# SandeepaInduwaraSamaranayake/SwinVox

Measured on AMD Instinct MI355X. Metric: views/sec fwd+bwd SwinVox-T 224^2, 32^3 voxel, n_views=8, higher is better.
Workload: dtype bf16; 1 GPU; SwinVox-T full pipeline (ResNet50[:layer3] || Swin multi-stage, cross-view attention, decoder, merger, refiner), fwd+2xBCE+bwd, train mode, B=64 samples x V=8 views of 224x224 per GPU; global_batch=64, n_views=8, images_per_gpu=512, parallelism=single GPU, launch=eager (one host launch per kernel, three streams)

## Files before the change

include/swinvox_hip.h:

```cpp
#ifndef SWINVOX_HIP_H
#define SWINVOX_HIP_H
#include <stddef.h>
#include <stdint.h>

#ifdef __cplusplus
extern "C" {
#endif

#define SV_OK 0
#define SV_ERR_INVALID (-1)
#define SV_ERR_LAUNCH (-2)

enum { SV_ACT_NONE = 0, SV_ACT_RELU = 1, SV_ACT_GELU = 2, SV_ACT_LRELU = 3 };
#define SV_BN_SLOTS 16
enum { SV_MATH_F32 = 0, SV_MATH_BF16 = 1, SV_MATH_FP8 = 2, SV_MATH_FP8_FULL = 3 };
enum { SV_F32 = 0, SV_BF16 = 1 };

const char* sv_last_error(void);
int sv_version(void);

typedef struct sv_geom {
  int N;
  int Di, Hi, Wi;
  int Do, Ho, Wo;
  int Ci, Co;
  int kd, kh, kw;
  int sd, sh, sw;
  int pd, ph, pw;
  int ldi;
} sv_geom;

typedef struct sv_epilogue {
  const float* bias;
  const void* residual;
  int ldr;
  const float* row_scale;
  int rows_per_scale;
  void* pre_act;
  double* stats;
  int act;
  float slope;
  const void* act_grad_src;
  int act_grad_kind;
  int ldc;
  int col_off;
} sv_epilogue;

int sv_conv_gather(const void* in, const void* w_packed, void* out, const sv_geom* g, const sv_epilogue* e,
                   int math, int act_dtype, void* stream);
int sv_set_conv_halo(int mode);
int sv_conv_halo_mode(void);
int sv_set_conv_halo_wgrad(int mode);
long long sv_conv_halo_launches(void);
enum { SV_PATH_GATHER = 0,
       SV_PATH_DENSE = 1,
       SV_PATH_WIDE = 2,
       SV_PATH_WIDE_GENERAL = 3,
       SV_PATH_HALO0 = 4, SV_PATH_HALO1 = 5, SV_PATH_HALO2 = 6,
       SV_PATH_HALO_BLOCKED_8X32 = 7, SV_PATH_HALO_BLOCKED_16X16 = 8,
       SV_PATH_WGRAD_TILED = 9,
       SV_PATH_WGRAD_WIDE = 10, SV_PATH_WGRAD_WIDE_SWAP = 11,
       SV_PATH_WGRAD_HALO = 12 };
enum { SV_OPERANDS_F32 = 0, SV_OPERANDS_BF16_F32 = 1, SV_OPERANDS_BF16 = 2 };
typedef struct sv_launch_plan {
  int path;
  int tile_rows, tile_cols;
  int operands;
  int vec;
  int grid_x, grid_y, block;
} sv_launch_plan;
int sv_conv_gather_plan(const void* in, const void* w, void* out, const sv_geom* g, const sv_epilogue* e, int math, int act_dtype, int transposed,
                        sv_launch_plan* plan);
int sv_conv_gather_is_wide(const void* in, const void* w, void* out, const sv_geom* g, const sv_epilogue* e, int math, int act_dtype);
int sv_tconv_gather(const void* in, const void* w_packed, void* out, const sv_geom* g, const sv_epilogue* e,
                    int math, int act_dtype, void* stream);
int sv_conv_wgrad_plan(const void* anchor, int lda, const void* gathered, const sv_geom* g, int cg_valid, int math, int act_dtype,
                       sv_launch_plan* plan);
int sv_conv_wgrad_is_wide(const void* anchor, int lda, const void* gathered, const sv_geom* g, int cg_valid, int math, int act_dtype);
size_t sv_conv_wgrad_workspace_floats(const sv_geom* g);
int sv_conv_wgrad(const void* anchor, int lda, const void* gathered, float* dw, const sv_geom* g, int cg_valid,
                  float* workspace, float* dbias , int math, int act_dtype,
                  void* stream);
int sv_quant_rows_e4m3(const void* src, int src_dtype, int rows, int K, int ld, void* dst_q, int Kp, float* scales, void* stream);
int sv_linear_fp8(const void* xq, const float* sx, const void* wq, const float* sw, void* out, int M, int K, int N, const sv_epilogue* e,
                  int act_dtype, void* stream);
int sv_linear_fp8_supported(int K, int N, const sv_epilogue* e, int math, int act_dtype);
long long sv_linear_fp8_launches(void);
int sv_quant_cols_e4m3(const void* src, int src_dtype, int M, int C, int ld, void* dst_q, int Mp, float* scales, float* colsum, void* stream);
int sv_linear_fp8_dgrad(const void* dq, const float* sd, const void* wtq, const float* swt, void* dx, int M, int N, int K, const sv_epilogue* e,
                        int act_dtype, void* stream);
int sv_linear_fp8_dgrad_supported(int N, int K, const sv_epilogue* e, int math, int act_dtype);
int sv_linear_fp8_wgrad(const void* dyt, const float* sdc, const void* xt, const float* sxc, float* dw, int M, int N, int K, int ldw, int splits,
                        void* stream);
long long sv_linear_fp8_bwd_launches(int which);
int sv_quant_rows_mx_e4m3(const void* src, int src_dtype, int rows, int K, int ld, void* dst_q, int Kp, void* scales_u8, void* stream);
int sv_linear_mxfp8(const void* xq, const void* xs, const void* wq, const void* ws, void* out, int M, int K, int N, const sv_epilogue* e,
                    void* q_out, void* qs_out, int act_dtype, void* stream);
long long sv_linear_mxfp8_launches(void);
long long sv_quant_rows_mx_launches(void);
int sv_quant_cols_mx_e4m3(const void* src, int src_dtype, int M, int C, int ld, void* dst_q, int Mp, void* scales_u8, float* colsum, void* stream);
int sv_linear_mxfp8_dgrad(const void* dq, const void* ds, const void* wtq, const void* wts, void* dx, int M, int N, int K, const sv_epilogue* e,
                          int act_dtype, void* stream);
size_t sv_linear_mxfp8_wgrad_workspace_floats(int M, int N, int K, int splits);
int sv_linear_mxfp8_wgrad(const void* dyt, const void* dys, const void* xt, const void* xs, float* dw, int M, int N, int K, int ldw, int splits,
                          float* workspace, void* stream);
long long sv_linear_mxfp8_bwd_launches(int which);
long long sv_quant_cols_mx_launches(void);
int sv_mx_rows_to_cols(const void* xq, int Kp, const void* xs, int M, int K, void* dst_q, int Mp, void* scales_u8, void* stream);
long long sv_mx_rows_to_cols_launches(void);
int sv_quant_rows_cols_mx_e4m3(const void* src, int src_dtype, int M, int N, int ld, void* row_q, int Np, void* row_s, void* col_q, int Mp,
                               void* col_s, float* colsum, void* stream);
long long sv_quant_rows_cols_mx_launches(void);
int sv_stencil3_fwd(const void* x, int ldx, int cin_load, int groups, const void* w_bf16, int ntiles16,
                    const float* bias, void* out, int ldc, int col_off, int cout, const void* residual, int ldr,
                    double* stats, int I, int D, int H, int W, long long x_plane_stride, long long out_plane_stride, int act_dtype,
                    void* stream);
size_t sv_stencil3_wgrad_workspace_floats(int cout, int cin);
int sv_stencil3_wgrad(const void* x, int ldx, int cin_load, int groups, const void* dy, int lddy, int cout_load,
                      float* dw, float* dbias, float* workspace, int cout, int cin, int c_stride, int c_valid, int I, int D, int H, int W,
                      long long x_plane_stride, int act_dtype, void* stream);
int sv_tconv4s2_fwd(const void* x, const void* w_packed, const float* bias, void* out, double* stats, int I, int D, int H, int W,
                    int cin, int cout, void* stream);
int sv_pack_weight(const float* src, void* dst, int A, int B, int T, int swap, int pad_to, int out_dtype, void* stream);
typedef struct sv_pack_desc {
  const float* src; void* dst;
  int A, B, T, swap, rows_out, inner_out, block0, reserved;
} sv_pack_desc;
int sv_pack_weights_block_elems(void);
int sv_pack_weights(const sv_pack_desc* descs_dev, int n, int total_blocks, int out_dtype, void* stream);
int sv_colsum(const void* x, int rows, int cols, int ld, float* out, int accumulate, int act_dtype, void* stream);
int sv_cast(const void* src, int src_dtype, void* dst, int dst_dtype, long long n, void* stream);

int sv_layernorm_fwd(const void* x, const float* gamma, const float* beta, void* y, float* mean, float* rstd,
                     long long rows, int C, float eps, int merge_H, int merge_W, int act_dtype, void* stream);
int sv_layernorm_quant_fwd(const void* x, const float* gamma, const float* beta, void* y, float* mean, float* rstd,
                           void* q, int Kp, float* scales, long long rows, int C, float eps, int merge_H, int merge_W,
                           int act_dtype, void* stream);
long long sv_layernorm_quant_launches(void);
int sv_layernorm_quant_mx_fwd(const void* x, const float* gamma, const float* beta, void* y, float* mean, float* rstd,
                              void* q, int Kp, void* scales_u8, long long rows, int C, float eps,
                              int merge_H, int merge_W, int act_dtype, void* stream);
long long sv_layernorm_quant_mx_launches(void);
size_t sv_layernorm_bwd_workspace_floats(int C);
int sv_layernorm_bwd(const void* dy, const void* x, const float* gamma, const float* mean, const float* rstd,
                     void* dx, float* dgamma, float* dbeta, float* workspace, long long rows, int C, int merge_H, int merge_W,
                     int accumulate_dx, int act_dtype, void* stream);
size_t sv_ln_image_workspace_floats(int I, int L);
int sv_ln_image_fwd(const void* x, const float* w, const float* b, void* y, float* meanrstd, float* workspace,
                    int I, int L, float eps, float drop_p, uint32_t seed, const uint32_t* seed_epoch, int act_dtype, void* stream);
int sv_ln_image_bwd(const void* dy, const void* x, const float* w, const float* meanrstd, void* dx, float* dw,
                    float* db, double* sums_ws , int I, int L, float drop_p, uint32_t seed,
                    const uint32_t* seed_epoch, int act_dtype, void* stream);
int sv_bn_stats(const void* x, long long M, int C, int ld, double* sums, int act_dtype, void* stream);
int sv_bn_finalize(const double* sums, long long count, const float* gamma, const float* beta, float* running_mean,
                   float* running_var, float momentum, float eps, int training, float* scale, float* shift,
                   float* save_mean, float* save_rstd, int C, void* stream);
int sv_scale_shift_act(const void* x, int ldx, const float* scale, const float* shift, const void* residual, int ldr,
                       void* y, int ldy, long long M, int C, int act, float slope, int act_dtype, void* stream);
int sv_bn_act_maxpool_fwd(const void* x, const float* scale, const float* shift, void* pooled, void* idx, int N, int H, int W, int C,
                          int act, float slope, int act_dtype, void* stream);
int sv_bn_maxpool_bwd(const void* dpooled, const void* idx, const void* x, const float* gamma, const float* save_mean, const float* save_rstd,
                      const float* fwd_scale, const float* fwd_shift, int N, int H, int W, int C, int act, float slope, int training,
                      void* dx, float* dgamma, float* dbeta, double* sums_ws, int act_dtype, void* stream);
int sv_bn_act_maxpool3d_fwd(const void* x, const float* scale, const float* shift, void* pooled, void* idx, int N, int D, int H, int W, int C,
                            int act, float slope, int act_dtype, void* stream);
// ... 153 lines not shown
```

swinvox_amd/hip.py:

```python
from __future__ import annotations

import ctypes as C
import os
import threading

import torch

_HERE = os.path.dirname(os.path.abspath(__file__))
LIB_PATH = os.environ.get("SV_HIP_LIB") or os.path.join(_HERE, "libswinvox_hip.so")

ACT_NONE, ACT_RELU, ACT_GELU, ACT_LRELU = 0, 1, 2, 3
MATH_F32, MATH_BF16, MATH_FP8, MATH_FP8_FULL = 0, 1, 2, 3
F32, BF16 = 0, 1


class Geom(C.Structure):
    _fields_ = [(n, C.c_int) for n in ("N", "Di", "Hi", "Wi", "Do", "Ho", "Wo", "Ci", "Co", "kd", "kh", "kw",
                                        "sd", "sh", "sw", "pd", "ph", "pw", "ldi")]


class Epilogue(C.Structure):
    _fields_ = [("bias", C.c_void_p), ("residual", C.c_void_p), ("ldr", C.c_int), ("row_scale", C.c_void_p),
                ("rows_per_scale", C.c_int), ("pre_act", C.c_void_p), ("stats", C.c_void_p), ("act", C.c_int),
                ("slope", C.c_float), ("act_grad_src", C.c_void_p), ("act_grad_kind", C.c_int), ("ldc", C.c_int),
                ("col_off", C.c_int)]


class LaunchPlan(C.Structure):
    _fields_ = [(n, C.c_int) for n in ("path", "tile_rows", "tile_cols", "operands", "vec", "grid_x", "grid_y", "block")]


(PATH_GATHER, PATH_DENSE, PATH_WIDE, PATH_WIDE_GENERAL, PATH_HALO0, PATH_HALO1, PATH_HALO2, PATH_HALO_BLOCKED_8X32, PATH_HALO_BLOCKED_16X16,
 PATH_WGRAD_TILED, PATH_WGRAD_WIDE, PATH_WGRAD_WIDE_SWAP, PATH_WGRAD_HALO) = range(13)
OPERANDS_F32, OPERANDS_BF16_F32, OPERANDS_BF16 = 0, 1, 2


class PackDesc(C.Structure):
    _fields_ = [("src", C.c_void_p), ("dst", C.c_void_p), ("A", C.c_int), ("B", C.c_int), ("T", C.c_int), ("swap", C.c_int),
                ("rows_out", C.c_int), ("inner_out", C.c_int), ("block0", C.c_int), ("reserved", C.c_int)]


class AugSample(C.Structure):
    _fields_ = [("bg", C.c_float * 3), ("jitter_value", C.c_float * 3), ("jitter_order", C.c_int * 3), ("noise", C.c_float * 3),
                ("perm", C.c_int * 3), ("mean", C.c_float * 3), ("std", C.c_float * 3)]


_P, _I, _L, _F, _U, _D = C.c_void_p, C.c_int, C.c_longlong, C.c_float, C.c_uint32, C.c_double
_ACT_TYPED = {
    "sv_conv_gather", "sv_tconv_gather", "sv_conv_wgrad", "sv_stencil3_fwd", "sv_stencil3_wgrad", "sv_colsum",
    "sv_layernorm_fwd", "sv_layernorm_quant_fwd", "sv_layernorm_quant_mx_fwd", "sv_layernorm_bwd", "sv_ln_image_fwd", "sv_ln_image_bwd", "sv_bn_stats", "sv_scale_shift_act", "sv_bn_bwd", "sv_scale_shift_act_signs", "sv_bn_bwd_signs", "sv_scale_shift_act2_signs", "sv_bn_bwd2_signs",
    "sv_window_attention_fwd", "sv_window_attention_fwd_mxq", "sv_window_attention_bwd", "sv_cross_view_attention_fwd", "sv_cross_view_attention_bwd",
    "sv_transpose", "sv_add_n", "sv_axpby", "sv_relu_bwd", "sv_maxpool2d_fwd", "sv_maxpool2d_bwd", "sv_avgpool2_fwd", "sv_avgpool2_bwd",
    "sv_decoder_seed_fwd", "sv_decoder_seed_bwd", "sv_maxpool3d_fwd", "sv_maxpool3d_bwd", "sv_dropout", "sv_rowscale",
    "sv_dwconv2x2_fwd", "sv_dwconv2x2_bwd", "sv_upsample3to7_add_fwd", "sv_upsample3to7_bwd",
    "sv_cva_downsample_fwd", "sv_cva_downsample_bwd", "sv_cva_upsample_add_fwd", "sv_cva_upsample_bwd", "sv_decoder_head_fwd", "sv_decoder_head_bwd",
    "sv_merge_views_fwd", "sv_merge_views_bwd", "sv_stem_space_to_depth", "sv_encoder_prep", "sv_encoder_prep_bwd", "sv_bn_act_maxpool_fwd", "sv_bn_maxpool_bwd", "sv_bn_act_maxpool3d_fwd", "sv_bn_maxpool3d_bwd", "sv_head_pack_x", "sv_head_unpack_dx", "sv_swin_attn_block_fwd", "sv_swin_attn_block_fwd_mx", "sv_swin_attn_block_bwd",
    "sv_linear_fp8", "sv_linear_fp8_dgrad", "sv_linear_mxfp8", "sv_linear_mxfp8_dgrad",
}
_PROTOS = {
    "sv_version": (_I, None),
    "sv_conv_gather": (_I, [_P, _P, _P, C.POINTER(Geom), C.POINTER(Epilogue), _I]),
    "sv_tconv_gather": (_I, [_P, _P, _P, C.POINTER(Geom), C.POINTER(Epilogue), _I]),
    "sv_conv_gather_plan": (_I, None, [_P, _P, _P, C.POINTER(Geom), C.POINTER(Epilogue), _I, _I, _I, C.POINTER(LaunchPlan)]),
    "sv_conv_gather_is_wide": (_I, None, [_P, _P, _P, C.POINTER(Geom), C.POINTER(Epilogue), _I, _I]),
    "sv_conv_wgrad_plan": (_I, None, [_P, _I, _P, C.POINTER(Geom), _I, _I, _I, C.POINTER(LaunchPlan)]),
    "sv_conv_wgrad_is_wide": (_I, None, [_P, _I, _P, C.POINTER(Geom), _I, _I, _I]),
    "sv_conv_wgrad_workspace_floats": (C.c_size_t, None, [C.POINTER(Geom)]),
    "sv_conv_wgrad": (_I, [_P, _I, _P, _P, C.POINTER(Geom), _I, _P, _P, _I]),
    "sv_quant_rows_e4m3": (_I, [_P, _I, _I, _I, _I, _P, _I, _P]),
    "sv_linear_fp8": (_I, [_P, _P, _P, _P, _P, _I, _I, _I, C.POINTER(Epilogue)]),
    "sv_linear_fp8_supported": (_I, None, [_I, _I, C.POINTER(Epilogue), _I, _I]),
    "sv_linear_fp8_launches": (_L, None),
    "sv_quant_cols_e4m3": (_I, [_P, _I, _I, _I, _I, _P, _I, _P, _P]),
    "sv_linear_fp8_dgrad": (_I, [_P, _P, _P, _P, _P, _I, _I, _I, C.POINTER(Epilogue)]),
    "sv_linear_fp8_dgrad_supported": (_I, None, [_I, _I, C.POINTER(Epilogue), _I, _I]),
    "sv_linear_fp8_wgrad": (_I, [_P, _P, _P, _P, _P, _I, _I, _I, _I, _I]),
    "sv_linear_fp8_bwd_launches": (_L, None, [_I]),
    "sv_quant_rows_mx_e4m3": (_I, [_P, _I, _I, _I, _I, _P, _I, _P]),
    "sv_linear_mxfp8": (_I, [_P, _P, _P, _P, _P, _I, _I, _I, C.POINTER(Epilogue), _P, _P]),
    "sv_linear_mxfp8_launches": (_L, None),
    "sv_quant_rows_mx_launches": (_L, None),
    "sv_quant_cols_mx_e4m3": (_I, [_P, _I, _I, _I, _I, _P, _I, _P, _P]),
    "sv_linear_mxfp8_dgrad": (_I, [_P, _P, _P, _P, _P, _I, _I, _I, C.POINTER(Epilogue)]),
    "sv_linear_mxfp8_wgrad_workspace_floats": (C.c_size_t, None, [_I, _I, _I, _I]),
    "sv_linear_mxfp8_wgrad": (_I, [_P, _P, _P, _P, _P, _I, _I, _I, _I, _I, _P]),
    "sv_linear_mxfp8_bwd_launches": (_L, None, [_I]),
    "sv_quant_cols_mx_launches": (_L, None),
    "sv_mx_rows_to_cols": (_I, [_P, _I, _P, _I, _I, _P, _I, _P]),
    "sv_mx_rows_to_cols_launches": (_L, None),
    "sv_quant_rows_cols_mx_e4m3": (_I, [_P, _I, _I, _I, _I, _P, _I, _P, _P, _I, _P, _P]),
    "sv_quant_rows_cols_mx_launches": (_L, None),
    "sv_stencil3_fwd": (_I, [_P, _I, _I, _I, _P, _I, _P, _P, _I, _I, _I, _P, _I, _P, _I, _I, _I, _I, _L, _L]),
    "sv_stencil3_wgrad_workspace_floats": (C.c_size_t, None, [_I, _I]),
    "sv_stencil3_wgrad": (_I, [_P, _I, _I, _I, _P, _I, _I, _P, _P, _P, _I, _I, _I, _I, _I, _I, _I, _I, _L]),
    "sv_tconv4s2_fwd": (_I, [_P, _P, _P, _P, _P, _I, _I, _I, _I, _I, _I]),
    "sv_pack_weight": (_I, [_P, _P, _I, _I, _I, _I, _I, _I]),
    "sv_pack_weights_block_elems": (_I, None),
    "sv_pack_weights": (_I, [_P, _I, _I, _I]),
    "sv_colsum": (_I, [_P, _I, _I, _I, _P, _I]),
    "sv_cast": (_I, [_P, _I, _P, _I, _L]),
    "sv_layernorm_fwd": (_I, [_P, _P, _P, _P, _P, _P, _L, _I, _F, _I, _I]),
    "sv_layernorm_quant_fwd": (_I, [_P, _P, _P, _P, _P, _P, _P, _I, _P, _L, _I, _F, _I, _I]),
    "sv_layernorm_quant_launches": (_L, None),
    "sv_layernorm_quant_mx_fwd": (_I, [_P, _P, _P, _P, _P, _P, _P, _I, _P, _L, _I, _F, _I, _I]),
    "sv_layernorm_quant_mx_launches": (_L, None),
    "sv_layernorm_bwd_workspace_floats": (C.c_size_t, None, [_I]),
    "sv_layernorm_bwd": (_I, [_P, _P, _P, _P, _P, _P, _P, _P, _P, _L, _I, _I, _I, _I]),
    "sv_bn_bwd_workspace_doubles": (C.c_size_t, None, [_I]),
    "sv_ln_image_workspace_floats": (C.c_size_t, None, [_I, _I]),
    "sv_ln_image_fwd": (_I, [_P, _P, _P, _P, _P, _P, _I, _I, _F, _F, _U, _P]),
    "sv_ln_image_bwd": (_I, [_P, _P, _P, _P, _P, _P, _P, _P, _I, _I, _F, _U, _P]),
    "sv_bn_stats": (_I, [_P, _L, _I, _I, _P]),
    "sv_bn_finalize": (_I, [_P, _L, _P, _P, _P, _P, _F, _F, _I, _P, _P, _P, _P, _I]),
    "sv_scale_shift_act": (_I, [_P, _I, _P, _P, _P, _I, _P, _I, _L, _I, _I, _F]),
    "sv_bn_bwd": (_I, [_P, _I, _P, _I, _P, _I, _P, _P, _P, _L, _I, _I, _F, _I, _P, _I, _P, _I, _P, _P, _P, _P, _P]),
    "sv_bn_signs_supported": (_I, None, [_I]),
    "sv_scale_shift_act_signs": (_I, [_P, _I, _P, _P, _P, _I, _P, _I, _L, _I, _I, _F, _P]),
    "sv_bn_bwd_signs": (_I, [_P, _I, _P, _P, _I, _P, _P, _P, _L, _I, _I, _F, _I, _P, _I, _P, _I, _P, _P, _P]),
    "sv_scale_shift_act2_signs": (_I, [_P, _I, _P, _P, _P, _I, _P, _P, _P, _I, _L, _I, _P]),
    "sv_bn_bwd2_signs": (_I, [_P, _I, _P, _P, _I, _P, _P, _P, _P, _I, _P, _P, _P, _L, _I, _P, _I, _P, _I, _P, _P, _P, _P, _P, _P]),
    "sv_window_attention_fwd": (_I, [_P, _P, _P, _I, _I, _I, _I, _I, _I, _I]),
    "sv_window_attention_fwd_mxq": (_I, [_P, _P, _P, _I, _I, _I, _I, _I, _I, _I, _P, _I, _P]),
    "sv_window_attention_bwd_workspace_floats": (C.c_size_t, None, [_I]),
    "sv_window_attention_windows_per_group": (_I, None, [_I, _I, _I, _I, _I, _I]),
    "sv_window_attention_bwd": (_I, [_P, _P, _P, _P, _P, _P, _I, _I, _I, _I, _I, _I, _I]),
    "sv_stem_space_to_depth": (_I, [_P, _P, _I]),
    "sv_bn_act_maxpool_fwd": (_I, [_P, _P, _P, _P, _P, _I, _I, _I, _I, _I, _F]),
    "sv_bn_maxpool_bwd": (_I, [_P, _P, _P, _P, _P, _P, _P, _P, _I, _I, _I, _I, _I, _F, _I, _P, _P, _P, _P]),
    "sv_bn_act_maxpool3d_fwd": (_I, [_P, _P, _P, _P, _P, _I, _I, _I, _I, _I, _I, _F]),
    "sv_bn_maxpool3d_bwd": (_I, [_P, _P, _P, _P, _P, _P, _P, _P, _I, _I, _I, _I, _I, _I, _F, _I, _P, _P, _P, _P]),
    "sv_set_conv_halo": (_I, None, [_I]),
    "sv_conv_halo_mode": (_I, None),
    "sv_set_conv_halo_wgrad": (_I, None, [_I]),
    "sv_conv_halo_launches": (_L, None),
    "sv_encoder_prep": (_I, [_P, _I, _P, _P, _I, _I]),
    "sv_encoder_prep_bwd": (_I, [_P, _P, _P, _I, _I, _I]),
    "sv_head_pack_x": (_I, [_P, _P, _I, _I]),
    "sv_head_unpack_dx": (_I, [_P, _P, _I, _I]),
    "sv_stem_pack": (_I, [_P, _P, _I]),
    "sv_stem_unpack_grad": (_I, [_P, _P]),
    "sv_stem_native": (_I, [_P, _P]),
    "sv_merger_pack": (_I, [_P, _P, _I, _I, _I, _I]),
    "sv_swin_mlp_supported": (_I, None, [_I]),
    "sv_swin_mlp_pack": (_I, [_P, _P, _P, _I]),
    "sv_swin_mlp_fwd": (_I, [_P, _P, _P, _P, _P, _P, _P, _P, _I, _L, _I, _F]),
    "sv_swin_mlp_bwd": (_I, [_P, _P, _P, _P, _P, _P, _P, _P, _I, _P, _P, _L, _I, _F]),
    "sv_swin_mlp_wgrad": (_I, [_P, _P, _P, _P, _P, _P, _P, _P, _I, _P, _P, _P, _P, _L, _I, _F]),
    "sv_swin_mlp_mx_supported": (_I, None, [_I]),
    "sv_swin_mlp_mx_pack_bytes": (_L, None, [_I]),
    "sv_swin_mlp_mx_pack": (_I, [_P, _P, _P, _P, _P, _I]),
    "sv_swin_mlp_fwd_mx": (_I, [_P, _P, _P, _P, _P, _P, _P, _P, _I, _L, _I, _F]),
# ... 197 lines not shown
```

swinvox_amd/models/_base.py:

```python
from __future__ import annotations

import math
from typing import Dict, List, Sequence

import torch
import torch.nn as nn

from .. import hip, ops
from ..ops import ACT_LRELU, ACT_NONE, ACT_RELU, BatchNormState, ConvSpec, call, empty, ptr, zeros


class GradStore:

    def __init__(self, params: Sequence[torch.Tensor], layout=None):
        from ..optim import FlatLayout
        self.params = list(params)
        self._map: Dict[int, torch.Tensor] = {}
        self.flat = None
        if self.params:
            layout = layout if layout is not None else FlatLayout(self.params)
            self.flat = torch.zeros(layout.total, dtype=torch.float32, device=self.params[0].device)
            for p, v in zip(self.params, layout.views(self.flat)):
                self._map[id(p)] = v

# ... 68 lines not shown
        if not views[0].is_cuda:
            hook(group_index, views)
            return
        cur = torch.cuda.current_stream()
        cs = ops.comm_stream(views[0].device)
        cs.wait_stream(cur)
        aw = ops._CTX.awg
        if aw is not None:
            cs.wait_stream(aw.stream)
        with torch.cuda.stream(cs):
            hook(group_index, views)

    def _grad_groups_cached(self):
        pl = self._param_list()
        gg = self.__dict__.get("_ggroups")
        if gg is None or gg[0] != len(pl):
            gg = self.__dict__["_ggroups"] = (len(pl), self.grad_groups())
        return gg[1]

    def _param_list(self) -> List[torch.Tensor]:
        pl = self.__dict__.get("_plist")
        if pl is None or len(pl) != self.__dict__.get("_plist_n", -1):
            pl = list(self.parameters())
            self.__dict__["_plist"], self.__dict__["_plist_n"] = pl, len(pl)
        return pl

    def _grad_layout(self):
        from ..optim import FlatLayout
        pl = self._param_list()
        lay = self.__dict__.get("_glayout")
        if lay is None or not lay.matches(pl):
            lay = self.__dict__["_glayout"] = FlatLayout(pl)
        return lay

    def _run(self, *inputs):
        hip.check_cuda(*inputs)
        hip.check_cuda(*self._param_list()[:1])
        for t in inputs:
            if t.dtype != torch.float32 and t.dtype != ops._STATE["store"]:
                raise RuntimeError(f"swinvox_amd: expected float32 inputs, got {t.dtype}")
        params = self._param_list()
        save = torch.is_grad_enabled() and (any(p.requires_grad for p in params) or any(t.requires_grad for t in inputs))
        return _ModuleFn.apply(self, len(inputs), save, *inputs, *params)

    def _seed(self) -> int:
        return int(torch.randint(0, 2 ** 31 - 1, (1,)).item())


LayerTape = ops.named_tape("LayerTape", "x ldi y st n in_grid M og z ldz idx w")


class ConvBnAct:

    def __init__(self, conv: nn.Module, bn: nn.Module, spec: ConvSpec, act: int, slope: float = 0.0):
        self.conv, self.bn, self.spec, self.act, self.slope = conv, bn, spec, act, slope

    def forward_stats(self, x, n, in_grid, training, *, ldi=None, w=None):
        sp = self.spec
        og = sp.out_grid(in_grid)
        M = n * og[0] * og[1] * og[2]
        y = empty(M, sp.cout, like=x)
        st = BatchNormState(self.bn, M, training)
        sp.forward(x, n, in_grid, self._pack("f") if w is None else w, y, ldi=ldi, bias=self.conv.bias, stats=st.sums)
        st.finalize()
        return LayerTape(x, ldi, y, st, n, in_grid, M, og, None, None, None, None)

    def forward(self, x, n, in_grid, training, *, ldi=None, z=None, ldz=None, residual=None, ldr=0):
        t = self.forward_stats(x, n, in_grid, training, ldi=ldi)
        C = self.spec.cout
        if z is None:
            z, ldz = empty(t.M, C, like=x), C
        t.st.apply(t.y, C, z, ldz, self.act, self.slope, residual, ldr)
        return z, t.og, t._replace(z=z if residual is not None else None, ldz=ldz)

    def backward(self, t, dz, lddz, grads, *, need_dx=True, dres=None, lddres=0, dx=None, lddx=None, dx_epi=None):
        sp = self.spec
        dy = (zeros if sp.cout_mem != sp.cout else empty)(t.M, sp.cout_mem, like=dz)
        t.st.backward(dz, lddz, t.z, t.ldz, t.y, sp.cout, dy, sp.cout_mem, grads[self.bn.weight], grads[self.bn.bias], self.act, self.slope,
                      dres, lddres)
        return self.backward_conv(t, dy, grads, need_dx=need_dx, dx=dx, lddx=lddx, dx_epi=dx_epi)

    def backward_conv(self, t, dy, grads, *, need_dx=True, dx=None, lddx=None, dx_epi=None):
        sp, n, in_grid = self.spec, t.n, t.in_grid
        sp.wgrad(dy, t.x, n, in_grid, self._dw(grads), lddy=sp.cout_mem, ldx=t.ldi,
                 db=grads[self.conv.bias] if self.conv.bias is not None else None)
        if not need_dx:
            return None
        Min = n * in_grid[0] * in_grid[1] * in_grid[2]
        if dx is None:
            dx = (zeros if sp.cin_mem != sp.cin else empty)(Min, sp.cin_mem, like=dy)
            lddx = sp.cin_mem
        sp.dgrad(dy, n, in_grid, self._pack("d"), dx, lddy=sp.cout_mem, lddx=lddx, **(dx_epi or {}))
        return dx

    def forward_pool(self, x, n, in_grid, training, *, w=None):
        t = self.forward_stats(x, n, in_grid, training, w=w)
        C, st = self.spec.cout, t.st
        st.probe(t.y, C)
        dims = t.og[1:] if t.og[0] == 1 else t.og
        p = empty(n * math.prod(d // 2 for d in dims), C, like=x)
        idx = torch.empty(p.numel(), dtype=torch.uint8, device=x.device)
        call("sv_bn_act_maxpool_fwd" if len(dims) == 2 else "sv_bn_act_maxpool3d_fwd", ptr(t.y), ptr(st.scale), ptr(st.shift), ptr(p), ptr(idx),
             n, *dims, C, self.act, self.slope)
        return p, t.og, t._replace(idx=idx)

    def backward_pool_bn(self, t, dp, grads):
        sp, st = self.spec, t.st
        assert sp.cout_mem == sp.cout
        dy = empty(t.M, sp.cout, like=dp)
        ws = ops.bn_bwd_workspace(sp.cout, dp.device)
        dims = t.og[1:] if t.og[0] == 1 else t.og
        call("sv_bn_maxpool_bwd" if len(dims) == 2 else "sv_bn_maxpool3d_bwd", ptr(dp), ptr(t.idx), ptr(t.y), ptr(self.bn.weight), ptr(st.mean),
             ptr(st.rstd), ptr(st.scale), ptr(st.shift), t.n, *dims, sp.cout, self.act, self.slope, 1 if st.training else 0, ptr(dy),
             ptr(grads[self.bn.weight]), ptr(grads[self.bn.bias]), ptr(ws))
        return dy

    def backward_pool(self, t, dp, grads, *, need_dx=True):
        return self.backward_conv(t, self.backward_pool_bn(t, dp, grads), grads, need_dx=need_dx)

    def _pack(self, kind):
        return self.spec.pack_fwd(self.conv.weight) if kind == "f" else self.spec.pack_dgrad(self.conv.weight)

    def _dw(self, grads):
        return grads[self.conv.weight]


def conv_spec_of(m: nn.Module, **kw) -> ConvSpec:
    if isinstance(m, nn.Linear):
        return ConvSpec.linear(m.in_features, m.out_features)
    if isinstance(m, nn.Conv2d):
        assert m.groups == 1 and m.dilation == (1, 1)
        return ConvSpec.conv2d(m.in_channels, m.out_channels, m.kernel_size, m.stride, m.padding, **kw)
    if isinstance(m, nn.ConvTranspose3d):
        assert m.groups == 1 and m.output_padding == (0, 0, 0)
        return ConvSpec.conv3d(m.in_channels, m.out_channels, m.kernel_size, m.stride, m.padding, transposed=True, **kw)
    if isinstance(m, nn.Conv3d):
        assert m.groups == 1
        return ConvSpec.conv3d(m.in_channels, m.out_channels, m.kernel_size, m.stride, m.padding, **kw)
    raise TypeError(type(m))
```

swinvox_amd/ops.py:

```python
from __future__ import annotations

import ctypes as C
import os
import threading
from dataclasses import dataclass
from typing import Any, NamedTuple, Optional, Tuple

import torch

from . import hip
from .hip import ACT_GELU, ACT_LRELU, ACT_NONE, ACT_RELU, Epilogue, Geom, call, ptr

_STATE = {"math": hip.MATH_F32, "store": torch.float32}


class _CallContext(threading.local):
    packs = None
    arena = None
    awg = None
    bn_tick = None
    dyq = None


_CTX = _CallContext()
# ... 954 lines not shown

    def apply(self, x, ldx, y, ldy, act=ACT_NONE, slope=0.0, residual=None, ldr=0):
        self.probe(x, ldx)
        self.signs = None
        if (residual is not None and act != ACT_NONE and self.training and _bn_signs_on() and self.C % 256 == 0
                and self.C % 4 == 0 and ldx % 4 == 0 and ldy % 4 == 0 and ldr % 4 == 0):
            self.signs = torch.empty(self.M * (self.C // 64), dtype=torch.int64, device=x.device)
            call("sv_scale_shift_act_signs", ptr(x), ldx, ptr(self.scale), ptr(self.shift), ptr(residual), ldr, ptr(y), ldy, self.M, self.C, act, slope,
                 ptr(self.signs))
            return
        call("sv_scale_shift_act", ptr(x), ldx, ptr(self.scale), ptr(self.shift), ptr(residual), ldr, ptr(y), ldy, self.M, self.C, act, slope)

    def backward(self, dz, lddz, z, ldz, x, ldx, dx, lddx, dgamma, dbeta, act=ACT_NONE, slope=0.0, dres=None, lddres=0):
        ws = bn_bwd_workspace(self.C, dz.device)
        if getattr(self, "signs", None) is not None and dres is not None:
            call("sv_bn_bwd_signs", ptr(dz), lddz, ptr(self.signs), ptr(x), ldx, ptr(self.bn.weight), ptr(self.mean), ptr(self.rstd), self.M, self.C,
                 act, slope, 1 if self.training else 0, ptr(dx), lddx, ptr(dres), lddres, ptr(dgamma), ptr(dbeta), ptr(ws))
            return
        call("sv_bn_bwd", ptr(dz), lddz, ptr(z), ldz, ptr(x), ldx, ptr(self.bn.weight), ptr(self.mean), ptr(self.rstd), self.M, self.C,
             act, slope, 1 if self.training else 0, ptr(dx), lddx, ptr(dres), lddres, ptr(dgamma), ptr(dbeta), ptr(ws),
             ptr(self.scale), ptr(self.shift))


def bn_dual_enabled(training: bool, C: int, act: int) -> bool:
    on = _STATE.get("bn_dual", os.environ.get("SV_BN_DUAL", "1") != "0")
    return bool(on and training and act == ACT_RELU and _bn_signs_on() and C % 256 == 0)


def set_bn_dual(on: bool) -> None:
    _STATE["bn_dual"] = bool(on)


def bn_dual_apply(st3: "BatchNormState", x3, ldx3, std: "BatchNormState", xd, ldxd, y, ldy) -> None:
    std.probe(xd, ldxd)
    st3.probe(x3, ldx3)
    st3.signs = torch.empty(st3.M * (st3.C // 64), dtype=torch.int64, device=x3.device)
    call("sv_scale_shift_act2_signs", ptr(x3), ldx3, ptr(st3.scale), ptr(st3.shift), ptr(xd), ldxd, ptr(std.scale), ptr(std.shift), ptr(y), ldy,
         st3.M, st3.C, ptr(st3.signs))


def bn_dual_backward(st3: "BatchNormState", std: "BatchNormState", dz, lddz, x3, ldx3, xd, ldxd, dx3, lddx3, dxd, lddxd, grads) -> None:
    ws = bn_bwd_workspace(st3.C, dz.device, layers=2)
    call("sv_bn_bwd2_signs", ptr(dz), lddz, ptr(st3.signs), ptr(x3), ldx3, ptr(st3.bn.weight), ptr(st3.mean), ptr(st3.rstd),
         ptr(xd), ldxd, ptr(std.bn.weight), ptr(std.mean), ptr(std.rstd), st3.M, st3.C, ptr(dx3), lddx3, ptr(dxd), lddxd,
         ptr(grads[st3.bn.weight]), ptr(grads[st3.bn.bias]), ptr(grads[std.bn.weight]), ptr(grads[std.bn.bias]), ptr(ws[0]), ptr(ws[1]))


def _bn_signs_on() -> bool:
    return _STATE.get("bn_signs", os.environ.get("SV_BN_SIGNS", "1") != "0")


def set_bn_signs(on: bool) -> None:
    _STATE["bn_signs"] = bool(on)


def input_prep_enabled() -> bool:
    return _STATE.get("input_prep", os.environ.get("SV_INPUT_PREP", "1") != "0")


def set_input_prep(on: bool) -> None:
    _STATE["input_prep"] = bool(on)


def bn_pool_fused_enabled() -> bool:
    return _STATE.get("bn_pool_fused", os.environ.get("SV_BN_POOL_FUSED", "1") != "0")


def set_bn_pool_fused(on: bool) -> None:
    _STATE["bn_pool_fused"] = bool(on)


def set_conv_halo(mode: int) -> None:
    rc = hip.load().sv_set_conv_halo(int(mode))
    if rc != 0:
        raise RuntimeError(f"sv_set_conv_halo failed (rc={rc}): {hip.load().sv_last_error().decode()}")


def set_conv_halo_wgrad(mode: int) -> None:
    rc = hip.load().sv_set_conv_halo_wgrad(int(mode))
    if rc != 0:
        raise RuntimeError(f"sv_set_conv_halo_wgrad failed (rc={rc}): {hip.load().sv_last_error().decode()}")


def set_bn_probe(fn) -> None:
    _STATE["bn_probe"] = fn


def transpose(src, dst, batch, R, Cc, lds=None, ldd=None, sb=None, db=None):
    lds = lds or Cc
    ldd = ldd or R
    assert src.dtype == dst.dtype
    call("sv_transpose", ptr(src), ptr(dst), batch, R, Cc, lds, ldd, sb if sb is not None else R * lds, db if db is not None else Cc * ldd,
         act=hip.BF16 if src.dtype == torch.bfloat16 else hip.F32)
```

Before: 5072 views/s.

## Fuse dgrad and wgrad of 64->256 1x1 conv backward into one kernel

```diff
diff --git a/include/swinvox_hip.h b/include/swinvox_hip.h
--- a/include/swinvox_hip.h
+++ b/include/swinvox_hip.h
@@ -81,6 +81,13 @@
 int sv_conv_wgrad(const void* anchor, int lda, const void* gathered, float* dw, const sv_geom* g, int cg_valid,
                   float* workspace, float* dbias , int math, int act_dtype,
                   void* stream);
+int sv_conv1x1_bwd_supported(int cin, int cout, long long rows, int math, int act_dtype);
+long long sv_conv1x1_bwd_min_rows(void);
+int sv_set_conv1x1_bwd(int mode);
+int sv_conv1x1_bwd_mode(void);
+long long sv_conv1x1_bwd_launches(void);
+int sv_conv1x1_bwd(const void* dy, int lddy, const void* x, int ldx, const void* w_dgrad, void* dx, int lddx, float* dw, float* db,
+                   long long rows, int cin, int cout, const void* bn, int grid_cap, int act_dtype, void* stream);
 int sv_quant_rows_e4m3(const void* src, int src_dtype, int rows, int K, int ld, void* dst_q, int Kp, float* scales, void* stream);
 int sv_linear_fp8(const void* xq, const float* sx, const void* wq, const float* sw, void* out, int M, int K, int N, const sv_epilogue* e,
                   int act_dtype, void* stream);
diff --git a/swinvox_amd/csrc/conv1x1_bwd.hip b/swinvox_amd/csrc/conv1x1_bwd.hip
--- /dev/null
+++ b/swinvox_amd/csrc/conv1x1_bwd.hip
@@ -0,0 +1,195 @@
+#include "common.h"
+#include <stdlib.h>
+#include <atomic>
+#include <type_traits>
+
+namespace sv {
+
+constexpr int CB_CIN = 64, CB_COUT = 256, CB_ROWS = 64, CB_NTHR = 512, CB_GRID = 256;
+constexpr long long CB_MIN_ROWS = 131072;
+constexpr int CB_LDY = CB_COUT + 16, CB_LDX = CB_CIN + 16, CB_LDO = CB_CIN + 8;
+constexpr int CB_Y_BYTES = CB_ROWS * CB_LDY * 2, CB_X_BYTES = CB_ROWS * CB_LDX * 2, CB_O_BYTES = CB_ROWS * CB_LDO * 2;
+constexpr int CB_W_BYTES = CB_COUT * CB_CIN * 4;
+constexpr int CB_LDS_BYTES = CB_W_BYTES > CB_Y_BYTES + CB_X_BYTES + CB_O_BYTES ? CB_W_BYTES : CB_Y_BYTES + CB_X_BYTES + CB_O_BYTES;
+static_assert(CB_ROWS * (CB_COUT / 8) == 4 * CB_NTHR && CB_ROWS * (CB_CIN / 8) == CB_NTHR, "16-byte chunks of a panel per thread: 4 of dy, 1 of x");
+static_assert(CB_COUT * CB_CIN == 32 * CB_NTHR, "32 accumulators per lane");
+
+struct Conv1x1BwdArgs {
+  const __bf16* dy; int lddy; const __bf16* x; int ldx; const __bf16* wd; __bf16* dx; int lddx; float* dw; long long rows; int npanels;
+};
+struct CbStage { bf16x8 y[4]; bf16x8 x; };
+
+typedef __attribute__((address_space(3))) bf16x4 cb_lds_bf16x4;
+
+__global__ __launch_bounds__(CB_NTHR) void conv1x1_bwd_kernel(const Conv1x1BwdArgs p) {
+  __shared__ __attribute__((aligned(16))) unsigned char lds[CB_LDS_BYTES];
+  __bf16* const Ys = reinterpret_cast<__bf16*>(lds);
+  __bf16* const Xs = reinterpret_cast<__bf16*>(lds + CB_Y_BYTES);
+  __bf16* const Os = reinterpret_cast<__bf16*>(lds + CB_Y_BYTES + CB_X_BYTES);
+  const int tid = threadIdx.x, lane = tid & 63, wave = tid >> 6, lr = lane & 15, lg = lane >> 4;
+  const int rt = wave >> 1, ch = wave & 1;
+  const int y_r = tid >> 5, y_c = (tid & 31) * 8;
+  const int x_r = tid >> 3, x_c = (tid & 7) * 8;
+  const int step = gridDim.x;
+
+  bf16x8 wf[2][8];
+#pragma unroll
+  for (int nt = 0; nt < 2; ++nt)
+#pragma unroll
+    for (int ks = 0; ks < 8; ++ks)
+      wf[nt][ks] = *reinterpret_cast<const bf16x8*>(p.wd + (size_t)(ch * 32 + nt * 16 + lr) * CB_COUT + ks * 32 + lg * 8);
+
+  f32x4 dwacc[2][4];
+#pragma unroll
+  for (int mt = 0; mt < 2; ++mt)
+#pragma unroll
+    for (int nt = 0; nt < 4; ++nt) dwacc[mt][nt] = (f32x4){0.f, 0.f, 0.f, 0.f};
+
+  auto load = [&](CbStage& s, int panel) {
+    const long long r0 = (long long)panel * CB_ROWS, last = p.rows - 1;
+#pragma unroll
+    for (int i = 0; i < 4; ++i) {
+      const long long r = r0 + y_r + 16 * i;
+      s.y[i] = *reinterpret_cast<const bf16x8*>(p.dy + (size_t)(r < last ? r : last) * p.lddy + y_c);
+    }
+    const long long r = r0 + x_r;
+    s.x = *reinterpret_cast<const bf16x8*>(p.x + (size_t)(r < last ? r : last) * p.ldx + x_c);
+  };
+  auto stage = [&](const CbStage& s, int panel) {
+    const long long r0 = (long long)panel * CB_ROWS;
+    const bf16x8 zero = VecN<__bf16, 8>::zero();
+#pragma unroll
+    for (int i = 0; i < 4; ++i)
+      *reinterpret_cast<bf16x8*>(Ys + (y_r + 16 * i) * CB_LDY + y_c) = r0 + y_r + 16 * i < p.rows ? s.y[i] : zero;
+    *reinterpret_cast<bf16x8*>(Xs + x_r * CB_LDX + x_c) = r0 + x_r < p.rows ? s.x : zero;
+  };
+  auto compute = [&]() {
+    f32x4 acc[2] = {(f32x4){0.f, 0.f, 0.f, 0.f}, (f32x4){0.f, 0.f, 0.f, 0.f}};
+    const __bf16* arow = Ys + (rt * 16 + lr) * CB_LDY + lg * 8;
+#pragma unroll
+    for (int ks = 0; ks < 8; ++ks) {
+      const bf16x8 a = *reinterpret_cast<const bf16x8*>(arow + ks * 32);
+#pragma unroll
+      for (int nt = 0; nt < 2; ++nt) acc[nt] = __builtin_amdgcn_mfma_f32_16x16x32_bf16(wf[nt][ks], a, acc[nt], 0, 0, 0);
+    }
+#pragma unroll
+    for (int nt = 0; nt < 2; ++nt) {
+      bf16x4 o;
+      o[0] = (__bf16)acc[nt][0]; o[1] = (__bf16)acc[nt][1]; o[2] = (__bf16)acc[nt][2]; o[3] = (__bf16)acc[nt][3];
+      *reinterpret_cast<bf16x4*>(Os + (rt * 16 + lr) * CB_LDO + ch * 32 + nt * 16 + lg * 4) = o;
+    }
+    const int q = lr >> 2, pp = lr & 3;
+#pragma unroll
+    for (int ks = 0; ks < CB_ROWS / 32; ++ks) {
+      bf16x8 a[2], b[4];
+#pragma unroll
+      for (int mt = 0; mt < 2; ++mt) {
+        const __bf16* src = Ys + (ks * 32 + lg * 8 + q) * CB_LDY + wave * 32 + mt * 16 + pp * 4;
+        const bf16x4 lo = __builtin_amdgcn_ds_read_tr16_b64_v4bf16((cb_lds_bf16x4*)(src));
+        const bf16x4 hi = __builtin_amdgcn_ds_read_tr16_b64_v4bf16((cb_lds_bf16x4*)(src + 4 * CB_LDY));
+        a[mt] = __builtin_shufflevector(lo, hi, 0, 1, 2, 3, 4, 5, 6, 7);
+      }
+#pragma unroll
+      for (int nt = 0; nt < 4; ++nt) {
+        const __bf16* src = Xs + (ks * 32 + lg * 8 + q) * CB_LDX + nt * 16 + pp * 4;
+        const bf16x4 lo = __builtin_amdgcn_ds_read_tr16_b64_v4bf16((cb_lds_bf16x4*)(src));
+        const bf16x4 hi = __builtin_amdgcn_ds_read_tr16_b64_v4bf16((cb_lds_bf16x4*)(src + 4 * CB_LDX));
+        b[nt] = __builtin_shufflevector(lo, hi, 0, 1, 2, 3, 4, 5, 6, 7);
+      }
+#pragma unroll
+      for (int mt = 0; mt < 2; ++mt)
+#pragma unroll
+        for (int nt = 0; nt < 4; ++nt) dwacc[mt][nt] = __builtin_amdgcn_mfma_f32_16x16x32_bf16(a[mt], b[nt], dwacc[mt][nt], 0, 0, 0);
+    }
+  };
+  auto panel_step = [&](CbStage& s, int panel, auto more) {
+    stage(s, panel);
+    __syncthreads();
+    if constexpr (decltype(more)::value) {
+      __builtin_amdgcn_sched_barrier(0);
+      load(s, min(panel + 2 * step, p.npanels - 1));
+      __builtin_amdgcn_sched_barrier(0);
+    }
+    compute();
+    __syncthreads();
+    const long long r = (long long)panel * CB_ROWS + x_r;
+    if (r < p.rows) *reinterpret_cast<bf16x8*>(p.dx + (size_t)r * p.lddx + x_c) = *reinterpret_cast<const bf16x8*>(Os + x_r * CB_LDO + x_c);
+  };
+
+  CbStage s0, s1;
+  int panel = blockIdx.x;
+  __builtin_amdgcn_sched_barrier(0);
+  load(s0, panel);
+  __builtin_amdgcn_sched_barrier(0);
+  load(s1, min(panel + step, p.npanels - 1));
+  __builtin_amdgcn_sched_barrier(0);
+  for (; panel + step < p.npanels; panel += 2 * step) {
+    panel_step(s0, panel, std::true_type{});
+    panel_step(s1, panel + step, std::true_type{});
+  }
+  if (panel < p.npanels) panel_step(s0, panel, std::false_type{});
+
+  __syncthreads();
+  float* const Ws = reinterpret_cast<float*>(lds);
+#pragma unroll
+  for (int mt = 0; mt < 2; ++mt)
+#pragma unroll
+    for (int nt = 0; nt < 4; ++nt)
+#pragma unroll
+      for (int j = 0; j < 4; ++j) Ws[(wave * 32 + mt * 16 + lg * 4 + j) * CB_CIN + nt * 16 + lr] = dwacc[mt][nt][j];
+  __syncthreads();
+  const int e0 = (int)(blockIdx.x & 255u) * 64 + tid;
+#pragma unroll 4
+  for (int i = 0; i < CB_COUT * CB_CIN / CB_NTHR; ++i) {
+    const int e = (e0 + CB_NTHR * i) & (CB_COUT * CB_CIN - 1);
+    atomicAdd(p.dw + e, Ws[e]);
+  }
+}
+
+static std::atomic<int>& conv1x1_bwd_mode() {
+  static std::atomic<int> m{[] { const char* v = getenv("SV_CONV1X1_BWD"); const int k = v ? atoi(v) : 1; return k < 0 || k > 2 ? 1 : k; }()};
+  return m;
+}
+static std::atomic<long long> conv1x1_bwd_launches{0};
+
+static bool conv1x1_bwd_shape(int cin, int cout, int math, int act_dtype) {
+  return cin == CB_CIN && cout == CB_COUT && math == SV_MATH_BF16 && act_dtype == SV_BF16;
+}
+
+}
+
+extern "C" int sv_set_conv1x1_bwd(int mode) {
+  SV_REQUIRE(mode >= 0 && mode <= 2, "sv_set_conv1x1_bwd: mode %d (0 off, 1 by sv_conv1x1_bwd_supported, 2 every supported shape)", mode);
+  sv::conv1x1_bwd_mode().store(mode, std::memory_order_relaxed);
+  return SV_OK;
+}
+extern "C" int sv_conv1x1_bwd_mode(void) { return sv::conv1x1_bwd_mode().load(std::memory_order_relaxed); }
+extern "C" long long sv_conv1x1_bwd_min_rows(void) { return sv::CB_MIN_ROWS; }
+extern "C" long long sv_conv1x1_bwd_launches(void) { return sv::conv1x1_bwd_launches.load(std::memory_order_relaxed); }
+extern "C" int sv_conv1x1_bwd_supported(int cin, int cout, long long rows, int math, int act_dtype) {
+  return sv::conv1x1_bwd_shape(cin, cout, math, act_dtype) && rows >= sv::CB_MIN_ROWS ? 1 : 0;
+}
+
+extern "C" int sv_conv1x1_bwd(const void* dy, int lddy, const void* x, int ldx, const void* w_dgrad, void* dx, int lddx, float* dw, float* db,
+                              long long rows, int cin, int cout, const void* bn, int grid_cap, int act_dtype, void* stream) {
+  using namespace sv;
+  SV_REQUIRE(conv1x1_bwd_shape(cin, cout, SV_MATH_BF16, act_dtype), "sv_conv1x1_bwd: cin=%d cout=%d act_dtype=%d (64 -> 256 on bf16 storage only)",
+             cin, cout, act_dtype);
+  SV_REQUIRE(dy && x && w_dgrad && dx && dw, "sv_conv1x1_bwd: null pointer");
+  SV_REQUIRE(db == nullptr, "sv_conv1x1_bwd: no bias gradient (the layers it serves have no bias)");
+  SV_REQUIRE(bn == nullptr, "sv_conv1x1_bwd: bn must be NULL (reserved)");
+  SV_REQUIRE(rows >= 1 && rows <= (1ll << 31) - CB_ROWS, "sv_conv1x1_bwd: rows=%lld", rows);
+  SV_REQUIRE(lddy >= cout && ldx >= cin && lddx >= cin && !(lddy & 7) && !(ldx & 7) && !(lddx & 7),
+             "sv_conv1x1_bwd: lddy=%d ldx=%d lddx=%d (multiples of 8, >= the channel count)", lddy, ldx, lddx);
+  SV_REQUIRE(!(((uintptr_t)dy | (uintptr_t)x | (uintptr_t)w_dgrad | (uintptr_t)dx) & 15) && !((uintptr_t)dw & 3), "sv_conv1x1_bwd: pointers must be 16-byte aligned");
+  SV_REQUIRE(grid_cap >= 0, "sv_conv1x1_bwd: grid_cap=%d", grid_cap);
+  const int npanels = (int)((rows + CB_ROWS - 1) / CB_ROWS);
+  int grid = npanels < CB_GRID ? npanels : CB_GRID;
+  if (grid_cap > 0 && grid > grid_cap) grid = grid_cap;
+  const Conv1x1BwdArgs a{static_cast<const __bf16*>(dy), lddy, static_cast<const __bf16*>(x), ldx, static_cast<const __bf16*>(w_dgrad),
+                         static_cast<__bf16*>(dx), lddx, dw, rows, npanels};
+  hipLaunchKernelGGL(conv1x1_bwd_kernel, dim3(grid), dim3(CB_NTHR), 0, static_cast<hipStream_t>(stream), a);
+  const int rc = check_launch("sv_conv1x1_bwd");
+  if (rc == SV_OK) conv1x1_bwd_launches.fetch_add(1, std::memory_order_relaxed);
+  return rc;
+}
diff --git a/swinvox_amd/hip.py b/swinvox_amd/hip.py
--- a/swinvox_amd/hip.py
+++ b/swinvox_amd/hip.py
@@ -47,7 +47,7 @@
 
 _P, _I, _L, _F, _U, _D = C.c_void_p, C.c_int, C.c_longlong, C.c_float, C.c_uint32, C.c_double
 _ACT_TYPED = {
-    "sv_conv_gather", "sv_tconv_gather", "sv_conv_wgrad", "sv_stencil3_fwd", "sv_stencil3_wgrad", "sv_colsum",
+    "sv_conv_gather", "sv_tconv_gather", "sv_conv_wgrad", "sv_conv1x1_bwd", "sv_stencil3_fwd", "sv_stencil3_wgrad", "sv_colsum",
     "sv_layernorm_fwd", "sv_layernorm_quant_fwd", "sv_layernorm_quant_mx_fwd", "sv_layernorm_bwd", "sv_ln_image_fwd", "sv_ln_image_bwd", "sv_bn_stats", "sv_scale_shift_act", "sv_bn_bwd", "sv_scale_shift_act_signs", "sv_bn_bwd_signs", "sv_scale_shift_act2_signs", "sv_bn_bwd2_signs",
     "sv_window_attention_fwd", "sv_window_attention_fwd_mxq", "sv_window_attention_bwd", "sv_cross_view_attention_fwd", "sv_cross_view_attention_bwd",
     "sv_transpose", "sv_add_n", "sv_axpby", "sv_relu_bwd", "sv_maxpool2d_fwd", "sv_maxpool2d_bwd", "sv_avgpool2_fwd", "sv_avgpool2_bwd",
@@ -67,6 +67,12 @@
     "sv_conv_wgrad_is_wide": (_I, None, [_P, _I, _P, C.POINTER(Geom), _I, _I, _I]),
     "sv_conv_wgrad_workspace_floats": (C.c_size_t, None, [C.POINTER(Geom)]),
     "sv_conv_wgrad": (_I, [_P, _I, _P, _P, C.POINTER(Geom), _I, _P, _P, _I]),
+    "sv_conv1x1_bwd_supported": (_I, None, [_I, _I, _L, _I, _I]),
+    "sv_conv1x1_bwd_min_rows": (_L, None),
+    "sv_set_conv1x1_bwd": (_I, None, [_I]),
+    "sv_conv1x1_bwd_mode": (_I, None),
+    "sv_conv1x1_bwd_launches": (_L, None),
+    "sv_conv1x1_bwd": (_I, [_P, _I, _P, _I, _P, _P, _I, _P, _P, _L, _I, _I, _P, _I]),
     "sv_quant_rows_e4m3": (_I, [_P, _I, _I, _I, _I, _P, _I, _P]),
     "sv_linear_fp8": (_I, [_P, _P, _P, _P, _P, _I, _I, _I, C.POINTER(Epilogue)]),
     "sv_linear_fp8_supported": (_I, None, [_I, _I, C.POINTER(Epilogue), _I, _I]),
diff --git a/swinvox_amd/models/_base.py b/swinvox_amd/models/_base.py
--- a/swinvox_amd/models/_base.py
+++ b/swinvox_amd/models/_base.py
@@ -174,11 +174,16 @@
 
     def backward_conv(self, t, dy, grads, *, need_dx=True, dx=None, lddx=None, dx_epi=None):
         sp, n, in_grid = self.spec, t.n, t.in_grid
+        Min = n * in_grid[0] * in_grid[1] * in_grid[2]
+        if need_dx and not dx_epi and self.conv.bias is None and ops.conv1x1_bwd_enabled(sp, Min):
+            if dx is None:
+                dx, lddx = empty(Min, sp.cin_mem, like=dy), sp.cin_mem
+            ops.conv1x1_bwd(sp, dy, t.x, self._pack("d"), dx, self._dw(grads), Min, lddy=sp.cout_mem, ldx=t.ldi, lddx=lddx)
+            return dx
         sp.wgrad(dy, t.x, n, in_grid, self._dw(grads), lddy=sp.cout_mem, ldx=t.ldi,
                  db=grads[self.conv.bias] if self.conv.bias is not None else None)
         if not need_dx:
             return None
-        Min = n * in_grid[0] * in_grid[1] * in_grid[2]
         if dx is None:
             dx = (zeros if sp.cin_mem != sp.cin else empty)(Min, sp.cin_mem, like=dy)
             lddx = sp.cin_mem
diff --git a/swinvox_amd/ops.py b/swinvox_amd/ops.py
--- a/swinvox_amd/ops.py
+++ b/swinvox_amd/ops.py
@@ -1060,6 +1060,36 @@
         raise RuntimeError(f"sv_set_conv_halo_wgrad failed (rc={rc}): {hip.load().sv_last_error().decode()}")
 
 
+def set_conv1x1_bwd(mode: int) -> None:
+    rc = hip.load().sv_set_conv1x1_bwd(int(mode))
+    if rc != 0:
+        raise RuntimeError(f"sv_set_conv1x1_bwd failed (rc={rc}): {hip.load().sv_last_error().decode()}")
+
+
+def conv1x1_bwd_enabled(spec: "ConvSpec", rows: int) -> bool:
+    if (spec.cin, spec.cout, spec.taps) != (64, 256, 1) or spec.transposed or spec.s != (1, 1, 1) or spec.p != (0, 0, 0):
+        return False
+    if spec.cin_mem != spec.cin or spec.cout_mem != spec.cout:
+        return False
+    lib = hip.load()
+    mode = lib.sv_conv1x1_bwd_mode()
+    if mode == 0:
+        return False
+    return bool(lib.sv_conv1x1_bwd_supported(spec.cin, spec.cout, lib.sv_conv1x1_bwd_min_rows() if mode == 2 else rows, _STATE["math"], hip.ACT))
+
+
+def conv1x1_bwd(spec: "ConvSpec", dy, x, w_dgrad, dx, dw, rows, *, lddy=None, ldx=None, lddx=None, grid_cap=0) -> None:
+    args = (ptr(dy), lddy or spec.cout_mem, ptr(x), ldx or spec.cin_mem, ptr(w_dgrad), ptr(dx), lddx or spec.cin_mem, ptr(dw), None,
+            rows, spec.cin, spec.cout, None, grid_cap)
+    tr = hip.TRACE
+    if tr is None or "sv_conv1x1_bwd" not in tr.names:
+        return call("sv_conv1x1_bwd", *args)
+    tr.begin("sv_conv1x1_bwd", 4.0 * rows * spec.cin * spec.cout, 2.0 * rows * (spec.cout + 2 * spec.cin) + 4.0 * spec.cin * spec.cout,
+             tag=f"rows={rows} cin={spec.cin} cout={spec.cout}")
+    call("sv_conv1x1_bwd", *args)
+    tr.end()
+
+
 def set_bn_probe(fn) -> None:
     _STATE["bn_probe"] = fn
 
```

Result: no change. 5104 views/s, median of 6 (+0.6%).
